# giuspugl/COSMOMAP2

Hardware: NVIDIA B200
Metric: tod_samples_per_s_per_pcg_iter (higher is better)
Workload: dtype f64

## Files before the change

### cosmomap2_b200/_cabi.py

```python
import ctypes
import os

_HERE = os.path.dirname(os.path.abspath(__file__))
LIB_PATH = os.environ.get("CM2_LIB") or os.path.join(_HERE, "csrc", "libcosmomap2_b200.so")

_vp = ctypes.c_void_p
_i64 = ctypes.c_int64
_int = ctypes.c_int
_f64 = ctypes.c_double

SIGNATURES = {
    "cm2_version": (_int, []),
    "cm2_last_error": (ctypes.c_char_p, []),
    "cm2_device_info": (_int, [ctypes.POINTER(_int), ctypes.POINTER(_i64), ctypes.POINTER(_int)]),
    "cm2_launch_count": (_i64, []),
    "cm2_pointing_apply": (_int, [_vp, _vp, _vp, _i64, _int, _vp, _vp, _vp]),
    "cm2_pointing_apply_t": (_int, [_vp, _vp, _vp, _i64, _int, _vp, _vp, _i64, _vp]),
    "cm2_pointing_apply_t_sorted": (_int, [_vp, _vp, _vp, _vp, _int, _vp, _vp, _i64, _vp]),
    "cm2_hits_i64": (_int, [_vp, _i64, _i64, _vp, _vp]),
    "cm2_angles": (_int, [_vp, _i64, _vp, _vp, _vp]),
    "cm2_pix_narrow": (_int, [_vp, _i64, _vp, _vp]),
    "cm2_pix_widen": (_int, [_vp, _i64, _vp, _vp]),
    "cm2_weights_moments": (_int, [_vp, _vp, _vp, _vp, _vp, _i64, _i64, _vp, _i64, _int, _vp, _i64, _vp]),
    "cm2_weights_moments_sorted": (_int, [_vp, _vp, _vp, _vp, _vp, _vp, _i64, _i64, _vp, _int, _vp, _i64, _vp]),
    "cm2_weights_mask": (_int, [_vp, _i64, _int, _f64, _vp, _vp]),
    "cm2_scan_scratch_bytes": (_i64, [_i64]),
    "cm2_weights_old2new": (_int, [_vp, _i64, _vp, _vp, _vp, _vp]),
    "cm2_compact_rows_f64": (_int, [_vp, _vp, _i64, _int, _vp, _vp]),
    "cm2_compact_rows_i64": (_int, [_vp, _vp, _i64, _int, _vp, _vp]),
    "cm2_relabel": (_int, [_vp, _i64, _vp, _vp]),
    "cm2_bd_build": (_int, [_vp, _i64, _int, _vp, _vp]),
    "cm2_bd_apply": (_int, [_vp, _i64, _int, _vp, _vp, _vp]),
    "cm2_bdfwd_apply": (_int, [_vp, _i64, _int, _vp, _vp, _vp]),
    "cm2_noise_white_apply": (_int, [_vp, _i64, _i64, _vp, _vp, _vp, _i64, _vp]),
    "cm2_toeplitz_scratch_bytes": (_i64, [_i64]),
    "cm2_noise_toeplitz_apply": (_int, [_vp, _int, _i64, _i64, _vp, _vp, _vp, _i64, _vp, _vp]),
    "cm2_toeplitz_fft_points": (_int, []),
    "cm2_toeplitz_fft_scratch_bytes": (_i64, [_i64]),
    "cm2_noise_toeplitz_fft_apply": (_int, [_vp, _int, _i64, _i64, _vp, _vp, _vp, _i64, _vp, _int, _int, _vp]),
    "cm2_filter_offset_apply": (_int, [_vp, _vp, _vp, _i64, _vp, _vp, _i64, _vp]),
    "cm2_amatvec_white": (_int, [_vp, _vp, _vp, _i64, _int, _vp, _i64, _i64, _vp, _vp, _vp, _i64, _i64, _vp]),
    "cm2_amatvec_white_set_stage": (_int, [_int]),
    "cm2_amatvec_filter": (_int, [_vp, _vp, _vp, _i64, _int, _vp, _vp, _i64, _vp, _vp, _i64, _vp]),
    "cm2_filter_runs_mark": (_int, [_vp, _vp, _vp, _i64, _i64, _vp, _vp, _vp]),
    "cm2_filter_runs_fill": (_int, [_vp, _vp, _vp, _int, _vp, _vp, _i64, _vp, _vp, _vp, _vp, _vp, _vp]),
    "cm2_filter_seg_mean": (_int, [_vp, _vp, _vp, _vp, _i64, _int, _vp, _vp, _vp]),
    "cm2_amatvec_filter_mu": (_int, [_vp, _vp, _vp, _i64, _int, _vp, _vp, _vp, _vp, _vp, _i64, _vp, _vp, _i64, _i64, _vp]),
    "cm2_filter_poly_gram": (_int, [_vp, _vp, _vp, _i64, _int, _vp, _vp, _vp]),
    "cm2_filter_poly_runs_fill": (_int, [_vp, _vp, _vp, _int, _vp, _vp, _i64, _int, _vp, _vp, _vp, _vp, _vp, _vp]),
    "cm2_filter_poly_seg_coef": (_int, [_vp, _vp, _vp, _vp, _i64, _int, _int, _vp, _vp, _vp, _vp]),
    "cm2_amatvec_filter_poly_mu": (_int, [_vp, _vp, _vp, _i64, _int, _vp, _vp, _vp, _vp, _vp, _i64, _int, _vp, _vp,
                                          _i64, _int, _i64, _vp]),
    "cm2_pointing_filter_mu": (_int, [_vp, _vp, _vp, _i64, _int, _vp, _vp, _vp, _vp, _vp, _i64, _vp, _vp, _vp]),
    "cm2_amatvec_toeplitz_max_band": (_int, []),
    "cm2_amatvec_toeplitz": (_int, [_vp, _vp, _vp, _i64, _int, _vp, _int, _i64, _i64, _vp, _vp, _vp, _i64, _vp]),
    "cm2_filter_poly_max_order": (_int, []),
    "cm2_filter_poly_set_tma": (_int, [_int]),
    "cm2_filter_poly_apply": (_int, [_vp, _vp, _vp, _i64, _i64, _int, _int, _vp, _vp, _i64, _vp]),
    "cm2_amatvec_filter_poly_max_order": (_int, []),
    "cm2_amatvec_filter_poly": (_int, [_vp, _vp, _vp, _i64, _int, _vp, _vp, _i64, _i64, _int, _vp, _vp, _i64, _vp]),
    "cm2_ground_filter_apply": (_int, [_vp, _i64, _i64, _vp, _vp, _vp, _vp, _vp]),
    "cm2_ground_filter_sub": (_int, [_vp, _i64, _i64, _vp, _vp, _vp, _vp, _vp]),
    "cm2_reorganize_map": (_int, [_vp, _vp, _i64, _int, _i64, _vp, _vp]),
    "cm2_defl_work_doubles": (_i64, [_int]),
    "cm2_defl_zt_apply": (_int, [_vp, _i64, _int, _i64, _vp, _int, _i64, _vp, _vp, _vp]),
    "cm2_defl_z_apply": (_int, [_vp, _i64, _int, _i64, _vp, _f64, _f64, _vp, _vp, _vp]),
    "cm2_coarse_apply": (_int, [_vp, _int, _vp, _vp, _vp]),
    "cm2_m2_apply": (_int, [_vp, _vp, _i64, _int, _i64, _vp, _vp, _i64, _int, _vp, _vp, _vp, _vp]),
    "cm2_m2_banded_apply": (_int, [_vp, _vp, _int, _vp, _vp, _i64, _int, _vp, _vp, _vp, _vp]),
    "cm2_dense_gram_work_doubles": (_i64, []),
    "cm2_dense_gram": (_int, [_vp, _i64, _int, _vp, _i64, _int, _i64, _vp, _i64, _vp, _vp]),
    "cm2_dense_combine": (_int, [_vp, _i64, _i64, _int, _vp, _i64, _int, _vp, _i64, _vp]),
    "cm2_dot": (_int, [_vp, _vp, _i64, _vp, _vp]),
    "cm2_axpby": (_int, [_f64, _vp, _f64, _vp, _i64, _vp]),
    "cm2_pcg_reset": (_int, [_vp, _i64, _vp, _f64, _vp]),
    "cm2_pcg_update_p": (_int, [_vp, _vp, _vp, _i64, _vp, _vp]),
    "cm2_pcg_update_xr": (_int, [_vp, _vp, _vp, _vp, _i64, _vp, _vp]),
    "cm2_pcg_bd_reset": (_int, [_vp, _i64, _int, _vp, _vp, _vp, _f64, _f64, _vp, _vp, _vp, _vp]),
    "cm2_pcg_bd_iter": (_int, [_vp, _i64, _int, _vp, _vp, _vp, _vp, _vp, _vp, _vp]),
    "cm2_pcg_bd_update_p": (_int, [_vp, _vp, _i64, _vp, _vp]),
    "cm2_pcg_bd_update": (_int, [_vp, _i64, _int, _vp, _vp, _vp, _vp, _vp, _vp, _vp]),
    "cm2_allreduce_p2p_signal_bytes": (_i64, []),
    "cm2_allreduce_p2p": (_int, [_vp, _vp, _vp, _int, _int, _i64, ctypes.c_uint32, _vp]),
    "cm2_enable_peer_access": (_int, [_int]),
    "cm2_allreduce_p2p_set_timeout": (_f64, [_f64]),
    "cm2_pcg_bd_iter_refuse": (_int, [_int]),
    "cm2_pcg_bd_iter_max_npix": (_i64, [_int]),
    "cm2_pcg_bd_tail_strided": (_int, [_int]),
    "cm2_pcg_sharded_signal_bytes": (_i64, []),
    "cm2_pcg_sharded_work_doubles": (_i64, []),
    "cm2_pcg_bd_sharded": (_int, [_int, _int, _int, _int, _int, _vp, _vp, _vp, _vp, _vp, _vp, _vp, _vp, _vp, _vp, _vp,
                                  _vp, ctypes.c_uint32, _f64, _f64, _f64, _vp]),
}

# ... 46 lines not shown
```

### cosmomap2_b200/csrc/tod_pass.cu

```cuda
#include <cstdint>
#include <type_traits>

#include "cm2_common.cuh"

namespace cm2 {

constexpr int K = 8;
constexpr int TILE = 32 * K;
constexpr int BLOCK = 256;
constexpr unsigned FULL = 0xffffffffu;

struct BlockW {
    const double *w;
    int64_t nblocks;
    int64_t blocksize;
    const int64_t *start;
    uint64_t magic;
};

static BlockW make_blockw(const double *w, int64_t nblocks, int64_t blocksize, const int64_t *start) {
    BlockW bw{w, nblocks, blocksize, start, 0};
    if (start == nullptr && blocksize > 1) bw.magic = ~(uint64_t)0 / (uint64_t)blocksize + 1;
    return bw;
}
// ... 41 lines not shown
    __device__ __forceinline__ int64_t tile(int64_t v) const {
        if (S == 1) return v;
        const unsigned q = (unsigned)v / S, r = (unsigned)v - q * S;
        return (int64_t)r * T + q;
    }
    __device__ __forceinline__ int64_t next(int64_t v, int64_t step, int64_t ntiles, int64_t &t) const {
        const int64_t nv = count();
        for (; v < nv; v += step) {
            t = tile(v);
            if (t < ntiles) return v;
        }
        t = -1;
        return v;
    }
};

static TileOrder make_order(int64_t nt, int64_t nstreams) {
    const int64_t ntiles = (nt + TILE - 1) / TILE;
    TileOrder o{1u, (unsigned)ntiles};
    if (nstreams > 1 && nstreams <= 65536 && ntiles >= 4 * nstreams && ntiles < ((int64_t)1 << 31)) {
        o.S = (unsigned)nstreams;
        o.T = (unsigned)((ntiles + nstreams - 1) / nstreams);
    }
    return o;
}

enum Cache { STREAM, KEEP };

template <Cache CP = STREAM>
__device__ __forceinline__ void load_pix(const int32_t *__restrict__ pix, int64_t t0, int64_t nt, int (&p)[K]) {
    if (t0 + K <= nt) {
        I8 v = CP == KEEP ? ld_keep_i8(pix + t0) : ld_stream_i8(pix + t0);
#pragma unroll
        for (int j = 0; j < K; ++j) p[j] = v.v[j];
    } else {
#pragma unroll
        for (int j = 0; j < K; ++j) p[j] = (t0 + j < nt) ? (CP == KEEP ? pix[t0 + j] : ld_stream_i1(pix + t0 + j)) : -1;
    }
}

template <Cache CP = STREAM>
__device__ __forceinline__ void load_f64(const double *__restrict__ a, int64_t t0, int64_t nt, double (&c)[K]) {
    if (t0 + K <= nt) {
        D4 v0 = CP == KEEP ? ld_keep_d4(a + t0) : ld_stream_d4(a + t0);
        D4 v1 = CP == KEEP ? ld_keep_d4(a + t0 + 4) : ld_stream_d4(a + t0 + 4);
#pragma unroll
        for (int j = 0; j < 4; ++j) { c[j] = v0.v[j]; c[4 + j] = v1.v[j]; }
    } else {
#pragma unroll
        for (int j = 0; j < K; ++j) c[j] = (t0 + j < nt) ? (CP == KEEP ? a[t0 + j] : ld_stream_d1(a + t0 + j)) : 0.0;
    }
}

template <int POL, Cache CP = STREAM>
__device__ __forceinline__ void load_tod(const int32_t *__restrict__ pix, const double *__restrict__ cs,
                                         const double *__restrict__ sn, int64_t t0, int64_t nt, int (&p)[K],
                                         double (&c)[K], double (&s)[K]) {
    load_pix<CP>(pix, t0, nt, p);
    if (POL > 1) { load_f64<CP>(cs, t0, nt, c); load_f64<CP>(sn, t0, nt, s); }
}

template <int POL>
__device__ __forceinline__ void gather_x(const double *__restrict__ x, const int (&p)[K], double (&xv)[K][POL]) {
#pragma unroll
    for (int j = 0; j < K; ++j) {
        const bool nw = (j == 0) || (p[j] != p[j - 1]);
#pragma unroll
        for (int k = 0; k < POL; ++k) xv[j][k] = 0.0;
        if (nw && p[j] >= 0) {
            const double *xp = x + (int64_t)POL * p[j];
#pragma unroll
            for (int k = 0; k < POL; ++k) xv[j][k] = __ldg(xp + k);
        }
    }
#pragma unroll
    for (int j = 1; j < K; ++j) {
        if (p[j] == p[j - 1]) {
#pragma unroll
            for (int k = 0; k < POL; ++k) xv[j][k] = xv[j - 1][k];
        }
    }
}

template <int POL>
__device__ __forceinline__ double project(const double (&xv)[POL], double c, double s) {
    if constexpr (POL == 1) return xv[0];
    else if constexpr (POL == 2) return fma(xv[1], s, xv[0] * c);
    else return fma(xv[2], s, fma(xv[1], c, xv[0]));
}

template <int POL>
__device__ __forceinline__ double project(const double (&xv)[K][POL], const double (&c)[K], const double (&s)[K], int j) {
    return project<POL>(xv[j], POL > 1 ? c[j] : 0.0, POL > 1 ? s[j] : 0.0);
}

template <int POL>
__device__ __forceinline__ auto pt_contrib(const double (&v)[K], const double (&c)[K], const double (&s)[K]) {
    return [&v, &c, &s](int j, double (&o)[POL]) {
        if constexpr (POL == 1) { o[0] = v[j]; }
        else if constexpr (POL == 2) { o[0] = v[j] * c[j]; o[1] = v[j] * s[j]; }
        else { o[0] = v[j]; o[1] = v[j] * c[j]; o[2] = v[j] * s[j]; }
    };
}

template <int NV, int STRIDE>
__device__ __forceinline__ void emit(double *__restrict__ y, int pix, const double (&v)[NV]) {
    if (pix >= 0) {
        double *dst = y + (int64_t)STRIDE * pix;
#pragma unroll
        for (int k = 0; k < NV; ++k) atomicAdd(dst + k, v[k]);
    }
}
// ... 87 lines not shown
__device__ __forceinline__ void run_scatter(double *__restrict__ y, const int (&p)[K], F contrib) {
    RunState<NV> rs;
    run_compress<NV, STRIDE>(y, p, contrib, rs);
    run_merge<NV, STRIDE>(y, rs);
}

template <int POL>
__global__ void __launch_bounds__(BLOCK) k_pointing_apply(const int32_t *__restrict__ pix, const double *__restrict__ cs,
                                                          const double *__restrict__ sn, int64_t nt,
                                                          const double *__restrict__ x, double *__restrict__ d) {
    const int lane = threadIdx.x & 31;
    const int64_t nwarps = (int64_t)gridDim.x * (BLOCK / 32);
    const int64_t ntiles = (nt + TILE - 1) / TILE;
    for (int64_t tile = (int64_t)blockIdx.x * (BLOCK / 32) + (threadIdx.x >> 5); tile < ntiles; tile += nwarps) {
        const int64_t t0 = tile * TILE + (int64_t)lane * K;
        if (t0 >= nt) continue;
        int p[K];
        double c[K], s[K], xv[K][POL], out[K];
        load_tod<POL>(pix, cs, sn, t0, nt, p, c, s);
        gather_x<POL>(x, p, xv);
#pragma unroll
        for (int j = 0; j < K; ++j) out[j] = p[j] >= 0 ? project<POL>(xv, c, s, j) : 0.0;
        if (t0 + K <= nt) {
            D4 a, b;
#pragma unroll
            for (int j = 0; j < 4; ++j) { a.v[j] = out[j]; b.v[j] = out[4 + j]; }
            st_stream_d4(d + t0, a);
            st_stream_d4(d + t0 + 4, b);
        } else {
#pragma unroll
            for (int j = 0; j < K; ++j) if (t0 + j < nt) d[t0 + j] = out[j];
        }
    }
}

template <int POL>
__global__ void __launch_bounds__(BLOCK) k_pointing_apply_t(const int32_t *__restrict__ pix, const double *__restrict__ cs,
                                                            const double *__restrict__ sn, int64_t nt,
                                                            const double *__restrict__ d, double *__restrict__ y) {
    const int lane = threadIdx.x & 31;
    const int64_t nwarps = (int64_t)gridDim.x * (BLOCK / 32);
    const int64_t ntiles = (nt + TILE - 1) / TILE;
    for (int64_t tile = (int64_t)blockIdx.x * (BLOCK / 32) + (threadIdx.x >> 5); tile < ntiles; tile += nwarps) {
        const int64_t t0 = tile * TILE + (int64_t)lane * K;
        int p[K];
        double c[K], s[K], v[K];
        load_pix(pix, t0, nt, p);
        load_f64(d, t0, nt, v);
        if (POL > 1) { load_f64(cs, t0, nt, c); load_f64(sn, t0, nt, s); }
        run_scatter<POL, POL>(y, p, pt_contrib<POL>(v, c, s));
    }
}

template <int POL, bool ILV, bool WS = false>
__global__ void __launch_bounds__(BLOCK) k_amatvec_white(const int32_t *__restrict__ pix, const double *__restrict__ cs,
                                                         const double *__restrict__ sn, int64_t nt, BlockW bw, TileOrder ord,
                                                         const double *__restrict__ x, double *__restrict__ y) {
    const int lane = threadIdx.x & 31;
    const int64_t nwarps = (int64_t)gridDim.x * (BLOCK / 32);
    const int64_t ntiles = (nt + TILE - 1) / TILE;
    RunState<POL> rs = RunState<POL>::empty();
    const int64_t nv = ILV ? ord.count() : ntiles;
    for (int64_t vt = (int64_t)blockIdx.x * (BLOCK / 32) + (threadIdx.x >> 5); vt < nv; vt += nwarps) {
        int64_t tile = vt;
        if constexpr (ILV) {
            tile = ord.tile(vt);
            if (tile >= ntiles) continue;
        }
        const int64_t t0 = tile * TILE + (int64_t)lane * K;
        int p[K];
        double c[K], s[K];
        load_tod<POL>(pix, cs, sn, t0, nt, p, c, s);
        run_merge<POL, POL>(y, rs);
        double w[K], xv[K][POL], v[K];
        if constexpr (WS) load_f64(bw.w, t0, nt, w);
        gather_x<POL>(x, p, xv);
        if constexpr (!WS) chunk_weights(bw, t0 < nt ? t0 : nt - 1, nt, w);
#pragma unroll
        for (int j = 0; j < K; ++j) v[j] = w[j] * project<POL>(xv, c, s, j);
        run_compress<POL, POL>(y, p, pt_contrib<POL>(v, c, s), rs);
    }
    run_merge<POL, POL>(y, rs);
}

template <int POL>
__device__ __forceinline__ void stage_flush(double *__restrict__ sm, double *__restrict__ y, int64_t base, int len) {
    const int lane = threadIdx.x & 31;
    __syncwarp();
    for (int i = lane; i < len; i += 32) {
        const double v = sm[i];
        if (v != 0.0) {
            sm[i] = 0.0;
            atomicAdd(y + base + i, v);
        }
    }
    __syncwarp();
}

template <int POL>
__global__ void __launch_bounds__(BLOCK) k_amatvec_white_staged(const int32_t *__restrict__ pix, const double *__restrict__ cs,
                                                                const double *__restrict__ sn, int64_t nt, BlockW bw, TileOrder ord,
                                                                const double *__restrict__ x, double *__restrict__ y, int wpix) {
    extern __shared__ double stage_sm[];
    const int lane = threadIdx.x & 31;
    double *sm = stage_sm + (size_t)(threadIdx.x >> 5) * POL * wpix;
    for (int i = lane; i < POL * wpix; i += 32) sm[i] = 0.0;
    __syncwarp();
    const int64_t nwarps = (int64_t)gridDim.x * (BLOCK / 32);
    const int64_t ntiles = (nt + TILE - 1) / TILE;
    const int64_t nv = ord.count();
    int64_t base_prev = 0;
    int len_prev = 0;
    for (int64_t vt = (int64_t)blockIdx.x * (BLOCK / 32) + (threadIdx.x >> 5); vt < nv; vt += nwarps) {
        const int64_t tile = ord.tile(vt);
        if (tile >= ntiles) continue;
        const int64_t t0 = tile * TILE + (int64_t)lane * K;
        int p[K];
        double c[K], s[K];
        load_tod<POL>(pix, cs, sn, t0, nt, p, c, s);
        if (len_prev) stage_flush<POL>(sm, y, base_prev, len_prev);
        len_prev = 0;
        double w[K], xv[K][POL], v[K];
        gather_x<POL>(x, p, xv);
        chunk_weights(bw, t0 < nt ? t0 : nt - 1, nt, w);
#pragma unroll
        for (int j = 0; j < K; ++j) v[j] = w[j] * project<POL>(xv, c, s, j);
        int lo = INT32_MAX, hi = INT32_MIN;
#pragma unroll
        for (int j = 0; j < K; ++j) {
            if (p[j] >= 0) { lo = min(lo, p[j]); hi = max(hi, p[j]); }
        }
        lo = __reduce_min_sync(FULL, lo);
        hi = __reduce_max_sync(FULL, hi);
        if (hi < lo) continue;
        auto contrib = pt_contrib<POL>(v, c, s);
// ... 719 lines not shown
}

static int check_tod(const void *pix, const void *c, const void *s, int64_t nt, int pol) {
    if (nt < 0) return set_error(CM2_ERR_ARG, "nt < 0");
    if (pol < 1 || pol > 3) return set_error(CM2_ERR_ARG, "No valid polarization key set! pol=%d (1=I, 2=QU, 3=IQU)", pol);
    if (nt > 0 && pix == nullptr) return set_error(CM2_ERR_ARG, "pix is NULL");
    if (pol > 1 && nt > 0 && (c == nullptr || s == nullptr)) return set_error(CM2_ERR_ARG, "cos/sin required for pol>1");
    if (!aligned(pix, 32) || !aligned(c, 32) || !aligned(s, 32))
        return set_error(CM2_ERR_ARG, "TOD arrays must be 32-byte aligned");
    return CM2_OK;
}

}

using namespace cm2;

extern "C" int cm2_pointing_apply(const int32_t *pix, const double *c, const double *s, int64_t nt, int pol,
                                  const double *x, double *d, cm2_stream_t stream) {
    int rc = check_tod(pix, c, s, nt, pol);
    if (rc) return rc;
    CM2_REQUIRE(aligned(d, 32), "d must be 32-byte aligned");
    if (nt == 0) return CM2_OK;
    cudaStream_t st = as_stream(stream);
    return with_pol(pol, [&](auto P) { return launch_tod(k_pointing_apply<P>, tod_blocks(nt), 0, st, pix, c, s, nt, x, d); });
}

extern "C" int cm2_pointing_apply_t(const int32_t *pix, const double *c, const double *s, int64_t nt, int pol,
                                    const double *d, double *y, int64_t npix, cm2_stream_t stream) {
    int rc = check_tod(pix, c, s, nt, pol);
    if (rc) return rc;
    CM2_REQUIRE(aligned(d, 32), "d must be 32-byte aligned");
    CM2_REQUIRE(npix >= 0, "npix < 0");
    cudaStream_t st = as_stream(stream);
    CM2_CUDA(zero_fill(y, npix, pol, st));
    if (nt == 0 || npix == 0) return CM2_OK;
    return with_pol(pol, [&](auto P) { return launch_tod(k_pointing_apply_t<P>, tod_blocks(nt), 0, st, pix, c, s, nt, d, y); });
}

static int check_blocks(const double *wblk, int64_t nblocks, int64_t blocksize, const int64_t *blk_start) {
    if (wblk == nullptr) return CM2_OK;
    if (nblocks <= 0) return set_error(CM2_ERR_ARG, "nblocks must be > 0 when weights are given");
    if (blk_start == nullptr && blocksize <= 0) return set_error(CM2_ERR_ARG, "blocksize must be > 0");
    return CM2_OK;
}

static int g_white_stage_wpix = 0;

extern "C" int cm2_amatvec_white_set_stage(int wpix) {
    CM2_REQUIRE(wpix >= 0 && wpix <= 1024, "stage window must be 0..1024 pixels");
    g_white_stage_wpix = wpix;
    return CM2_OK;
}

extern "C" int cm2_amatvec_white(const int32_t *pix, const double *c, const double *s, int64_t nt, int pol,
                                 const double *wblk, int64_t nblocks, int64_t blocksize, const int64_t *blk_start,
                                 const double *x, double *y, int64_t npix, int64_t nstreams, cm2_stream_t stream) {
    int rc = check_tod(pix, c, s, nt, pol);
    if (rc) return rc;
    rc = check_blocks(wblk, nblocks, blocksize, blk_start);
    if (rc) return rc;
    CM2_REQUIRE(npix >= 0, "npix < 0");
    cudaStream_t st = as_stream(stream);
    CM2_CUDA(zero_fill(y, npix, pol, st));
    if (nt == 0 || npix == 0) return CM2_OK;
    const BlockW bw = make_blockw(wblk, nblocks, blocksize, blk_start);
    const TileOrder ord = make_order(nt, nstreams);
    if (g_white_stage_wpix > 0) {
        const int wpix = g_white_stage_wpix;
        const size_t smem = sizeof(double) * (size_t)(BLOCK / 32) * pol * wpix;
        return with_pol(pol, [&](auto P) {
            return launch_tod(k_amatvec_white_staged<P>, tod_blocks(nt), smem, st, pix, c, s, nt, bw, ord, x, y, wpix);
        });
    }
    if (wblk != nullptr && blk_start == nullptr && blocksize == 1) {
        CM2_REQUIRE(nblocks >= nt && aligned(wblk, 32), "per-sample weights: nt values, 32-byte aligned");
        return with_pol(pol, [&](auto P) {
            return launch_tod(k_amatvec_white<P, false, true>, tod_blocks(nt), 0, st, pix, c, s, nt, bw, ord, x, y);
        });
    }
    return with_pol(pol, [&](auto P) {
        return launch_tod(ord.S > 1 ? k_amatvec_white<P, true> : k_amatvec_white<P, false>, tod_blocks(nt), 0, st,
                          pix, c, s, nt, bw, ord, x, y);
    });
}

template <int POL, int NLAG>
static int launch_amatvec_toeplitz(const int32_t *pix, const double *c, const double *s, int64_t nt, const ToepW &tw,
                                   const double *x, double *y, cudaStream_t st) {
    constexpr int VAL = TILE - 2 * ((NLAG + K - 1) / K) * K;
    return launch_tod(k_amatvec_toeplitz<POL, NLAG>, tod_blocks(nt, VAL), 0, st, pix, c, s, nt, tw, x, y);
}

template <int POL>
static int dispatch_amatvec_toeplitz(const int32_t *pix, const double *c, const double *s, int64_t nt, const ToepW &tw,
                                     const double *x, double *y, cudaStream_t st) {
    const int nlag = tw.nband - 1;
    if (nlag <= 2) return launch_amatvec_toeplitz<POL, 2>(pix, c, s, nt, tw, x, y, st);
    if (nlag <= 4) return launch_amatvec_toeplitz<POL, 4>(pix, c, s, nt, tw, x, y, st);
    return launch_amatvec_toeplitz<POL, 8>(pix, c, s, nt, tw, x, y, st);
}

extern "C" int cm2_amatvec_toeplitz_max_band(void) { return 9; }

extern "C" int cm2_amatvec_toeplitz(const int32_t *pix, const double *c, const double *s, int64_t nt, int pol,
                                    const double *band, int nband, int64_t nblocks, int64_t blocksize,
                                    const int64_t *blk_start, const double *x, double *y, int64_t npix,
                                    cm2_stream_t stream) {
    int rc = check_tod(pix, c, s, nt, pol);
    if (rc) return rc;
    CM2_REQUIRE(band != nullptr && nband >= 1, "band required");
    rc = check_blocks(band, nblocks, blocksize, blk_start);
    if (rc) return rc;
    if (nband > cm2_amatvec_toeplitz_max_band())
        return set_error(CM2_ERR_UNSUPPORTED, "fused Toeplitz A-matvec: nband=%d, bands of up to %d coefficients are supported",
                         nband, cm2_amatvec_toeplitz_max_band());
    CM2_REQUIRE(npix >= 0, "npix < 0");
    cudaStream_t st = as_stream(stream);
    CM2_CUDA(zero_fill(y, npix, pol, st));
    if (nt == 0 || npix == 0) return CM2_OK;
    const ToepW tw{band, nband, make_blockw(nullptr, nblocks, blocksize, blk_start)};
    return with_pol(pol, [&](auto P) { return dispatch_amatvec_toeplitz<P>(pix, c, s, nt, tw, x, y, st); });
}

extern "C" int cm2_weights_moments(const int32_t *pix, const double *c, const double *s, const double *w,
                                   const double *wblk, int64_t nblocks, int64_t blocksize, const int64_t *blk_start,
                                   int64_t nt, int pol, double *mom, int64_t npix, cm2_stream_t stream) {
    int rc = check_tod(pix, c, s, nt, pol);
    if (rc) return rc;
    rc = check_blocks(wblk, nblocks, blocksize, blk_start);
    if (rc) return rc;
    CM2_REQUIRE(aligned(w, 32), "w must be 32-byte aligned");
    CM2_REQUIRE(npix >= 0, "npix < 0");
    cudaStream_t st = as_stream(stream);
    CM2_CUDA(zero_fill(mom, npix, 6, st));
    if (nt == 0 || npix == 0) return CM2_OK;
    const BlockW bw = make_blockw(wblk, nblocks, blocksize, blk_start);
// ... 117 lines not shown
```

### cosmomap2_b200/linearoperators.py

```python
import numpy as np
import torch
from scipy.linalg import eigh, lu_factor, lu_solve

from . import _device as dv
from . import linop as lp
from .process_ces import BlockWeights, ProcessTimeSamples


def _stream():
    return dv.stream()


class SparseLO(lp.LinearOperator):

    def __init__(self, n, m, pix_samples, pol=1, angle_processed=None):
        dv.require_cuda()
        self.ncols = int(n)
        self.nrows = int(m)
        self.pol = pol
        self.pairs = pix_samples
        if pol not in (1, 2, 3):
            raise RuntimeError("No valid polarization key set!\t=>\tpol=%d \n \
                                    Possible values are pol=%d(I),%d(QU), %d(IQU)." % (pol, 1, 2, 3))
        if len(pix_samples) != self.nrows:
# ... 428 lines not shown
                self.nseg, self._max_seg_len, self.poly_order, int(self._sorted), dv.ptr(d), dv.ptr(out),
                d.numel(), _stream())
        return out

    def mult(self, d):
        if FILTER_STAGED:
            return self._staged(d)
        out = torch.empty_like(d)
        dv.call("cm2_filter_offset_apply", dv.ptr(self._pix_dev), dv.ptr(self._seg_start), dv.ptr(self._seg_end),
                self.nseg, dv.ptr(d), dv.ptr(out), d.numel(), _stream())
        return out

    def polyfilter(self, d):
        return self._staged(d)

    polyfilter_multithreads = polyfilter

    def compute_legendres(self):
        from .utilities import get_legendre_polynomials
        sizes = []
        for array in self.subscans:
            for i in array:
                if int(i) not in sizes:
                    sizes.append(int(i))
        self._legendres = {size: get_legendre_polynomials(self.poly_order, size) for size in sizes}

    @property
    def legendres(self):
        if self._legendres is None:
            self.compute_legendres()
        return self._legendres


TOD_INTERLEAVE_MIN_MAP_BYTES = 100e6


def _tod_streams(P, samples_per_timeline):
    ns = int(samples_per_timeline or 0)
    if ns <= 0 or 2 * 8 * P.pol * P.ncols < TOD_INTERLEAVE_MIN_MAP_BYTES:
        return 1
    k = P.nrows // ns
    return int(k) if k > 1 and k * ns == P.nrows else 1


def _filter_timeline(F):
    ns = np.atleast_1d(np.asarray(F.nsamples)).astype(np.int64)
    return int(ns[0]) if ns.size and np.all(ns == ns[0]) else 0


WHITE_STAGE_RUN_RANGE = (3.0, 6.0)
WHITE_STAGE_MIN_CONTIGUITY = 0.9
WHITE_STAGE_WINDOW = 288
WHITE_SORT_BELOW_RUN = 3.0


class _FusedWhiteA(lp.LinearOperator):

    def __init__(self, P, N):
        self.P, self.N = P, N
        n = P.pol * P.ncols
        bs = N._blk.blocksize if N is not None else 0
        self._streams = _tod_streams(P, bs)
        self._mode = None
        self._sorted = None
        super(_FusedWhiteA, self).__init__(n, n, matvec=self._run, symmetric=True, device=True)

    def _choose(self):
        run, contig = self.P.run_statistics()
        if run < WHITE_SORT_BELOW_RUN and self.P.nrows > 0:
            self._mode = "sorted"
            self._build_sorted()
        elif WHITE_STAGE_RUN_RANGE[0] <= run < WHITE_STAGE_RUN_RANGE[1] and contig >= WHITE_STAGE_MIN_CONTIGUITY:
            self._mode = "staged"
        else:
            self._mode = "registers"

    def _build_sorted(self):
        P, N = self.P, self.N
        order = torch.sort(P._pix_dev, stable=True).indices
        nflag = int((P._pix_dev < 0).sum().item())
        order = order[nflag:]
        nts = int(order.numel())
        pad = (-nts) % 8
        pix = torch.full((nts + pad,), -1, dtype=torch.int32, device=order.device)
        pix[:nts] = P._pix_dev[order]
        cs = sn = None
        if P.pol > 1:
            cs, sn = dv.zeros_f64(nts + pad), dv.zeros_f64(nts + pad)
            cs[:nts] = P._cos_dev[order]
            sn[:nts] = P._sin_dev[order]
        w = None
        if N is not None:
            starts = dv.to_dev(N._blk.starts, torch.int64)
            blk = torch.bucketize(order, starts[1:], right=True)
            w = dv.zeros_f64(nts + pad)
            w[:nts] = N.weights_dev()[blk]
        self._sorted = (pix, cs, sn, w, nts + pad)

    def _run(self, x):
        P = self.P
        if self._mode is None:
            self._choose()
        y = dv.out_f64(P.ncols * P.pol)
        if self._mode == "sorted":
            pix, cs, sn, w, nts = self._sorted
            dv.call("cm2_amatvec_white", dv.ptr(pix), dv.ptr(cs), dv.ptr(sn), nts, P.pol,
                    dv.ptr(w) if w is not None else None, nts if w is not None else 0, 1, None, dv.ptr(x), dv.ptr(y),
                    P.ncols, 1, _stream())
            return y
        if self.N is None:
            w, nb, bs, startp = None, 0, 0, None
        else:
            w = dv.ptr(self.N.weights_dev())
            nb, bs, startp = self.N._blk.args()
        if self._mode == "staged":
            dv.call("cm2_amatvec_white_set_stage", WHITE_STAGE_WINDOW)
        try:
            dv.call("cm2_amatvec_white", dv.ptr(P._pix_dev), dv.ptr(P._cos_dev), dv.ptr(P._sin_dev), P.nrows, P.pol,
                    w, nb, bs, startp, dv.ptr(x), dv.ptr(y), P.ncols, self._streams, _stream())
        finally:
            if self._mode == "staged":
                dv.call("cm2_amatvec_white_set_stage", 0)
        return y


FILTER_RUN_TABLE = True


def _tile_tables(seg_start, seg_end, nseg, nt):
    dev = seg_start.device
    ntiles = (nt + 255) // 256
    tile_t0 = torch.arange(ntiles, dtype=torch.int64, device=dev) * 256
    tile_seg = torch.searchsorted(seg_end, tile_t0, right=True)
    kk = torch.clamp(tile_seg, max=nseg - 1)
    a, b = seg_start[kk], seg_end[kk]
    t1 = torch.clamp(tile_t0 + 256, max=nt)
    inside = (tile_seg < nseg) & (a <= tile_t0) & (t1 <= b)
    outside = (tile_seg >= nseg) | (a >= t1)
    tile_flag = torch.full((ntiles,), 2, dtype=torch.uint8, device=dev)
    tile_flag[inside] = 1
    tile_flag[outside] = 0
    return tile_seg.to(torch.int32), tile_flag


def _build_filter_runs(P, F):
    nt, st = P.nrows, _stream()
    dev = P._pix_dev.device
    ss, se = F._seg_start_host, F._seg_end_host
    if F.nseg == 0 or np.any(ss[1:] < se[:-1]):
        return False
    flags = torch.empty(max(nt, 1), dtype=torch.int32, device=dev)
    pixm = torch.empty(max(nt, 1), dtype=torch.int32, device=dev)
    dv.call("cm2_filter_runs_mark", dv.ptr(P._pix_dev), dv.ptr(F._seg_start), dv.ptr(F._seg_end), F.nseg, nt,
            dv.ptr(flags), dv.ptr(pixm), st)
    runidx = torch.empty(max(nt, 1), dtype=torch.int32, device=dev)
    count = torch.zeros(1, dtype=torch.int64, device=dev)
    scratch = torch.empty(int(dv.call("cm2_scan_scratch_bytes", nt)) // 8 + 1, dtype=torch.int64, device=dev)
    dv.call("cm2_weights_old2new", dv.ptr(flags), nt, dv.ptr(runidx), dv.ptr(count), dv.ptr(scratch), st)
    nruns = int(count.item())
    del flags, scratch
    if nruns == 0 or 2 * nruns > nt:
        return False
    run_pix = torch.empty(nruns, dtype=torch.int32, device=dev)
    run_mom = torch.empty(3 * nruns, dtype=torch.float64, device=dev)
    seg_first = torch.empty(max(F.nseg, 1), dtype=torch.int64, device=dev)
    seg_nruns = torch.empty(max(F.nseg, 1), dtype=torch.int32, device=dev)
    dv.call("cm2_filter_runs_fill", dv.ptr(pixm), dv.ptr(P._cos_dev), dv.ptr(P._sin_dev), P.pol,
            dv.ptr(F._seg_start), dv.ptr(F._seg_end), F.nseg, dv.ptr(runidx), dv.ptr(run_pix), dv.ptr(run_mom),
            dv.ptr(seg_first), dv.ptr(seg_nruns), st)
    del pixm, runidx
    tile_seg, tile_flag = _tile_tables(F._seg_start, F._seg_end, F.nseg, nt)
    mu = torch.empty(max(F.nseg, 1), dtype=torch.float64, device=dev)
# ... 541 lines not shown
```

### cosmomap2_b200/workloads.py

```python
import time

import numpy as np
import torch
import torch.distributed as dist


def _world():
    if dist.is_available() and dist.is_initialized():
        return dist.get_world_size(), dist.get_rank()
    return 1, 0


def _max_over_ranks(v):
    t = torch.tensor([float(v)], dtype=torch.float64, device="cuda")
    if _world()[0] > 1:
        dist.all_reduce(t, op=dist.ReduceOp.MAX)
    return float(t.item())


def _barrier():
    torch.cuda.synchronize()
    if _world()[0] > 1:
        dist.barrier()
        torch.cuda.synchronize()
# ... 295 lines not shown
    x_m2, _res, out["M_2lvl"] = _solve(cm, A, b, M2, rtol, maxiter)
    out["iteration_ratio"] = out["M_2lvl"]["iterations"] / max(out["M_BD"]["iterations"], 1)
    out["build_plus_solve_vs_M_BD_solve"] = (out["deflation"]["build_seconds"] + out["M_2lvl"]["seconds"]) / out["M_BD"]["seconds"]
    ax1, ax2 = A._apply(x_bd), A._apply(x_m2)
    out["Ax_agreement"] = float(torch.linalg.norm(ax1 - ax2) / torch.linalg.norm(ax1))
    for k in ("M_BD", "M_2lvl"):
        out[k]["samples_per_s_per_pcg_iter"] = nt * world / (out[k]["ms_per_iteration"] * 1e-3)
    al_ms = time_device(lambda: A_local._apply(x_bd), time_iters)
    m2_ms = time_device(lambda: M2._apply(x_bd), time_iters)
    out["A_local_apply_ms"] = al_ms
    out["M_2lvl_apply_ms"] = m2_ms
    out["roofline"] = _roofline("k_seg_mean + k_amatvec_filter_mu (P^T F P, cm2_amatvec_filter_mu)" if poly_order == 0
                                else "P^T F_K P (Legendre order %d)" % poly_order, 20.0 * nt + 48.0 * npix, al_ms,
                                note=("DRAM traffic of the pair measured by ncu at 1e8 samples, 8 samples per pixel crossing "
                                      "(profiles/r02_filter_mu_ncu.txt): 2.41 GB against 2.024 GB algorithmic -- k_amatvec_filter_mu "
                                      "reads 1.00x its 20 B/sample, the rest is the run table of k_seg_mean (28 B per run); "
                                      "not measured at this size, hence traffic = null") if poly_order == 0 else None)
    out["hbm_GB"] = torch.cuda.max_memory_allocated() / 1e9
    _close(A)
    return out


def white(nt=1e9, nside=2048, nx=3200, ny=1600, ndet=64, steps=30):
    import cosmomap2_b200 as cm
    from cosmomap2_b200 import distributed
    from cosmomap2_b200.pcg import make_solver
    world, rank = _world()
    pol = 3
    nt, ns, pix, phi, _sl, _ss, g = make_scan(int(nt), nside, nx, ny, ndet, 8.0, seed=rank, turnaround=0.0)
    npix_full = 12 * nside ** 2
    w = 0.5 + torch.rand(ndet, generator=g, device="cuda", dtype=torch.float64).cpu().numpy()
    N = cm.BlockLO(ns, w)
    pts = cm.ProcessTimeSamples(pix, npix_full, obspix=np.arange(npix_full), pol=pol, phi=phi, w=N.diag,
                                comm=(True if world > 1 else None))
    del phi
    npix = pts.get_new_pixel[0]
    n = pol * npix
    P = cm.SparseLO(npix, nt, pts._pix_dev, pol=pol, angle_processed=pts)
    Mbd = cm.BlockDiagonalPreconditionerLO(pts, npix, pol=pol)
    A_local = P.T * N * P
    A = distributed.AllReduceLO(A_local) if world > 1 else A_local
    b = torch.randn(n, dtype=torch.float64, device="cuda", generator=torch.Generator(device="cuda").manual_seed(5))
    b = A._apply(b)
    x, info = cm.cg(A, b, M=Mbd, rtol=1e-10, maxiter=20)
    relres = float(torch.linalg.norm(b - A._apply(x)) / torch.linalg.norm(b))
    solver = make_solver(A, Mbd, n)

    def one_step():
        solver.start(b)
        solver.step_async()
        solver.tick()
    it_ms = time_device(one_step, steps)
    al_ms = time_device(lambda: A_local._apply(x), steps)
    out = {"config": "configs[4]: white noise, IQU nside=%d, M_BD PCG" % nside, "world": world, "nt_total": nt * world,
           "nt_per_gpu": nt, "npix": int(npix), "nside": nside, "cg_info": int(info), "relres": relres,
           "ms_per_pcg_iteration": it_ms, "samples_per_s_per_pcg_iter": nt * world / (it_ms * 1e-3),
           "A_local_apply_ms": al_ms,
           "roofline": _roofline("k_amatvec_white<3> (cm2_amatvec_white)", 20.0 * nt + 48.0 * npix, al_ms),
           "solver": type(solver).__name__, "hbm_GB": torch.cuda.max_memory_allocated() / 1e9}
    _close(A)
    return out
```

### include/cosmomap2_b200.h

```cpp
#ifndef COSMOMAP2_B200_H
#define COSMOMAP2_B200_H

#include <stdint.h>

#ifdef __cplusplus
extern "C" {
#endif

#define CM2_OK 0
#define CM2_ERR_ARG (-1)
#define CM2_ERR_CUDA (-2)
#define CM2_ERR_UNSUPPORTED (-3)

typedef void *cm2_stream_t;

int cm2_version(void);
const char *cm2_last_error(void);
int cm2_device_info(int *sm_count, int64_t *l2_bytes, int *cc);
int64_t cm2_launch_count(void);

int cm2_pointing_apply(const int32_t *pix, const double *cos2phi, const double *sin2phi,
                       int64_t nt, int pol, const double *x, double *d, cm2_stream_t stream);
int cm2_pointing_apply_t(const int32_t *pix, const double *cos2phi, const double *sin2phi,
                         int64_t nt, int pol, const double *d, double *y, int64_t npix,
                         cm2_stream_t stream);
int cm2_pointing_apply_t_sorted(const int64_t *rowptr, const int32_t *perm,
                                const double *cos2phi, const double *sin2phi, int pol,
                                const double *d, double *y, int64_t npix, cm2_stream_t stream);
int cm2_hits_i64(const int32_t *pix, int64_t nt, int64_t npix, int64_t *hits,
                 cm2_stream_t stream);

int cm2_angles(const double *phi, int64_t nt, double *cos2phi, double *sin2phi,
               cm2_stream_t stream);
int cm2_pix_narrow(const int64_t *pix64, int64_t nt, int32_t *pix32, cm2_stream_t stream);
int cm2_pix_widen(const int32_t *pix32, int64_t nt, int64_t *pix64, cm2_stream_t stream);
int cm2_weights_moments(const int32_t *pix, const double *cos2phi, const double *sin2phi,
                        const double *w, const double *wblk, int64_t nblocks, int64_t blocksize,
                        const int64_t *blk_start, int64_t nt, int pol, double *mom, int64_t npix,
                        cm2_stream_t stream);
int cm2_weights_moments_sorted(const int64_t *rowptr, const int32_t *perm, const double *cos2phi,
                               const double *sin2phi, const double *w, const double *wblk,
                               int64_t nblocks, int64_t blocksize, const int64_t *blk_start,
                               int pol, double *mom, int64_t npix, cm2_stream_t stream);
int cm2_weights_mask(const double *mom, int64_t npix, int pol, double threshold_cond,
                     int32_t *good, cm2_stream_t stream);
int64_t cm2_scan_scratch_bytes(int64_t n);
int cm2_weights_old2new(const int32_t *good, int64_t npix, int32_t *old2new,
                        int64_t *npix_new_dev, void *scratch, cm2_stream_t stream);
int cm2_compact_rows_f64(const double *src, const int32_t *old2new, int64_t npix, int width,
                         double *dst, cm2_stream_t stream);
int cm2_compact_rows_i64(const int64_t *src, const int32_t *old2new, int64_t npix, int width,
                         int64_t *dst, cm2_stream_t stream);
int cm2_relabel(int32_t *pix, int64_t nt, const int32_t *old2new, cm2_stream_t stream);

int cm2_bd_build(const double *mom, int64_t npix, int pol, double *inv, cm2_stream_t stream);
int cm2_bd_apply(const double *inv, int64_t npix, int pol, const double *x, double *y,
                 cm2_stream_t stream);
int cm2_bdfwd_apply(const double *mom, int64_t npix, int pol, const double *x, double *y,
                    cm2_stream_t stream);

int cm2_noise_white_apply(const double *wblk, int64_t nblocks, int64_t blocksize,
                          const int64_t *blk_start, const double *d, double *out, int64_t nt,
                          cm2_stream_t stream);
int64_t cm2_toeplitz_scratch_bytes(int64_t nblocks);
int cm2_noise_toeplitz_apply(const double *band, int nband, int64_t nblocks, int64_t blocksize,
                             const int64_t *blk_start, const double *d, double *out, int64_t nt,
                             void *scratch, cm2_stream_t stream);
int cm2_toeplitz_fft_points(void);
int64_t cm2_toeplitz_fft_scratch_bytes(int64_t nblocks);
int cm2_noise_toeplitz_fft_apply(const double *coef, int nband, int64_t nblocks, int64_t blocksize,
                                 const int64_t *blk_start, const double *d, double *out,
                                 int64_t nt, void *scratch, int init, int pair, cm2_stream_t stream);
int cm2_filter_offset_apply(const int32_t *pix, const int64_t *seg_start, const int64_t *seg_end,
                            int64_t nseg, const double *d, double *out, int64_t nt,
                            cm2_stream_t stream);

int cm2_amatvec_white(const int32_t *pix, const double *cos2phi, const double *sin2phi,
                      int64_t nt, int pol, const double *wblk, int64_t nblocks,
                      int64_t blocksize, const int64_t *blk_start, const double *x, double *y,
                      int64_t npix, int64_t nstreams, cm2_stream_t stream);
int cm2_amatvec_white_set_stage(int wpix);
int cm2_amatvec_filter(const int32_t *pix, const double *cos2phi, const double *sin2phi,
                       int64_t nt, int pol, const int64_t *seg_start, const int64_t *seg_end,
                       int64_t nseg, const double *x, double *y, int64_t npix,
                       cm2_stream_t stream);

int cm2_filter_runs_mark(const int32_t *pix, const int64_t *seg_start, const int64_t *seg_end,
                         int64_t nseg, int64_t nt, int32_t *flags, int32_t *pix_masked,
                         cm2_stream_t stream);
int cm2_filter_runs_fill(const int32_t *pix_masked, const double *cos2phi, const double *sin2phi,
                         int pol, const int64_t *seg_start, const int64_t *seg_end, int64_t nseg,
                         const int32_t *runidx, int32_t *run_pix, double *run_mom,
                         int64_t *seg_first, int32_t *seg_nruns, cm2_stream_t stream);
int cm2_filter_seg_mean(const int32_t *run_pix, const double *run_mom, const int64_t *seg_first,
                        const int32_t *seg_nruns, int64_t nseg, int pol, const double *x,
                        double *mu, cm2_stream_t stream);
int cm2_amatvec_filter_mu(const int32_t *pix, const double *cos2phi, const double *sin2phi,
                          int64_t nt, int pol, const int64_t *seg_start, const int64_t *seg_end,
                          const double *seg_mu, const int32_t *tile_seg, const uint8_t *tile_flag,
                          int64_t nseg, const double *x, double *y, int64_t npix, int64_t nstreams,
                          cm2_stream_t stream);

int cm2_filter_poly_gram(const int32_t *pix, const int64_t *seg_start, const int64_t *seg_end,
                         int64_t nseg, int poly_order, double *W, double *info, cm2_stream_t stream);
int cm2_filter_poly_runs_fill(const int32_t *pix_masked, const double *cos2phi, const double *sin2phi,
                              int pol, const int64_t *seg_start, const int64_t *seg_end, int64_t nseg,
                              int poly_order, const int32_t *runidx, int32_t *run_pix, double *run_mom,
                              int64_t *seg_first, int32_t *seg_nruns, cm2_stream_t stream);
int cm2_filter_poly_seg_coef(const int32_t *run_pix, const double *run_mom, const int64_t *seg_first,
                             const int32_t *seg_nruns, int64_t nseg, int pol, int poly_order,
                             const double *W, const double *x, double *coef, cm2_stream_t stream);
int cm2_amatvec_filter_poly_mu(const int32_t *pix, const double *cos2phi, const double *sin2phi,
                               int64_t nt, int pol, const int64_t *seg_start, const int64_t *seg_end,
                               const double *seg_coef, const int32_t *tile_seg, const uint8_t *tile_flag,
                               int64_t nseg, int poly_order, const double *x, double *y, int64_t npix,
                               int accumulate, int64_t nstreams, cm2_stream_t stream);

int cm2_pointing_filter_mu(const int32_t *pix, const double *cos2phi, const double *sin2phi,
                           int64_t nt, int pol, const int64_t *seg_start, const int64_t *seg_end,
                           const double *seg_mu, const int32_t *tile_seg, const uint8_t *tile_flag,
                           int64_t nseg, const double *x, double *d, cm2_stream_t stream);

int cm2_amatvec_toeplitz_max_band(void);
int cm2_amatvec_toeplitz(const int32_t *pix, const double *cos2phi, const double *sin2phi,
                         int64_t nt, int pol, const double *band, int nband, int64_t nblocks,
                         int64_t blocksize, const int64_t *blk_start, const double *x, double *y,
                         int64_t npix, cm2_stream_t stream);

int64_t cm2_defl_work_doubles(int r);
int cm2_defl_zt_apply(const double *Z, int64_t n, int r, int64_t ldz, const double *X,
                      int ncols_x, int64_t ldx, double *out, double *work, cm2_stream_t stream);
int cm2_defl_z_apply(const double *Z, int64_t n, int r, int64_t ldz, const double *c,
                     double alpha, double beta, const double *y0, double *y,
// ... 76 lines not shown
```

Baseline: 243.1 billion.

## Pack pointing pixel indices into 8-byte words per lane for white matvec

Adds a one-time packing kernel that encodes each lane's K=8 pixel indices as a base, a 16-bit delta and 2-bit codes in one 64-bit word. Lanes that don't fit this encoding are marked as escapes and fall back to reading int32 pixels. The white-noise A matvec reads these packed words with an evict-first, L1 no-allocate streaming load and prefetches the next tile's word one iteration ahead. This cuts pixel-index HBM traffic from 4 to about 1 byte per sample, at the cost of decode ALU work and escape fallback reads. The packed path is only chosen for single-stream layouts with short runs and high contiguity.

```diff
diff --git a/cosmomap2_b200/_cabi.py b/cosmomap2_b200/_cabi.py
--- a/cosmomap2_b200/_cabi.py
+++ b/cosmomap2_b200/_cabi.py
@@ -39,7 +39,8 @@
     "cm2_toeplitz_fft_scratch_bytes": (_i64, [_i64]),
     "cm2_noise_toeplitz_fft_apply": (_int, [_vp, _int, _i64, _i64, _vp, _vp, _vp, _i64, _vp, _int, _int, _vp]),
     "cm2_filter_offset_apply": (_int, [_vp, _vp, _vp, _i64, _vp, _vp, _i64, _vp]),
-    "cm2_amatvec_white": (_int, [_vp, _vp, _vp, _i64, _int, _vp, _i64, _i64, _vp, _vp, _vp, _i64, _i64, _vp]),
+    "cm2_amatvec_white": (_int, [_vp, _vp, _vp, _vp, _i64, _int, _vp, _i64, _i64, _vp, _vp, _vp, _i64, _i64, _vp]),
+    "cm2_pack_pointing": (_int, [_vp, _i64, _vp, _vp, _vp]),
     "cm2_amatvec_white_set_stage": (_int, [_int]),
     "cm2_amatvec_filter": (_int, [_vp, _vp, _vp, _i64, _int, _vp, _vp, _i64, _vp, _vp, _i64, _vp]),
     "cm2_filter_runs_mark": (_int, [_vp, _vp, _vp, _i64, _i64, _vp, _vp, _vp]),
diff --git a/cosmomap2_b200/csrc/tod_pass.cu b/cosmomap2_b200/csrc/tod_pass.cu
--- a/cosmomap2_b200/csrc/tod_pass.cu
+++ b/cosmomap2_b200/csrc/tod_pass.cu
@@ -117,12 +117,71 @@
     }
 }
 
+constexpr int PK_FLAGGED = -1, PK_ESCAPE = -2;
+
+__device__ __forceinline__ uint64_t ld_stream_u64(const uint64_t *p) {
+    uint64_t pol, r;
+    asm("createpolicy.fractional.L2::evict_first.b64 %0, 1.0;" : "=l"(pol));
+    asm volatile("ld.global.L1::no_allocate.L2::cache_hint.b64 %0, [%1], %2;" : "=l"(r) : "l"(p), "l"(pol));
+    return r;
+}
+
+__device__ __forceinline__ uint64_t load_packed(const uint64_t *__restrict__ pk, int64_t t0, int64_t nt) {
+    return t0 + K <= nt ? ld_stream_u64(pk + t0 / K) : (uint64_t)(uint32_t)PK_ESCAPE;
+}
+
+__device__ __forceinline__ void unpack_pix(uint64_t wd, const int32_t *__restrict__ pix, int64_t t0, int64_t nt,
+                                           int (&p)[K]) {
+    const int b0 = (int)(uint32_t)wd;
+    if (b0 == PK_ESCAPE) {
+        load_pix(pix, t0, nt, p);
+        return;
+    }
+    const int b1 = b0 + (int)(int16_t)(uint16_t)(wd >> 32);
+    const unsigned codes = (unsigned)(wd >> 48);
+#pragma unroll
+    for (int j = 0; j < K; ++j) {
+        const unsigned code = (codes >> (2 * j)) & 3u;
+        p[j] = ((code & 2u) ? b1 : b0) + (int)(code & 1u);
+    }
+}
+
 template <int POL, Cache CP = STREAM>
 __device__ __forceinline__ void load_tod(const int32_t *__restrict__ pix, const double *__restrict__ cs,
                                          const double *__restrict__ sn, int64_t t0, int64_t nt, int (&p)[K],
                                          double (&c)[K], double (&s)[K]) {
     load_pix<CP>(pix, t0, nt, p);
     if (POL > 1) { load_f64<CP>(cs, t0, nt, c); load_f64<CP>(sn, t0, nt, s); }
+}
+
+__device__ __forceinline__ uint64_t pack_lane(const int (&q)[K]) {
+    bool all_flagged = true, any_flagged = false;
+    int b0 = q[0];
+#pragma unroll
+    for (int j = 0; j < K; ++j) {
+        all_flagged &= q[j] == -1;
+        any_flagged |= q[j] < 0;
+        b0 = min(b0, q[j]);
+    }
+    if (all_flagged) return (uint32_t)PK_FLAGGED;
+    if (any_flagged) return (uint32_t)PK_ESCAPE;
+    int b1 = b0;
+#pragma unroll
+    for (int j = 0; j < K; ++j) {
+        if (q[j] - b0 > 1 && (b1 == b0 || q[j] < b1)) b1 = q[j];
+    }
+    if (b1 - b0 > INT16_MAX) return (uint32_t)PK_ESCAPE;
+    uint64_t codes = 0;
+#pragma unroll
+    for (int j = 0; j < K; ++j) {
+        const int d0 = q[j] - b0, d1 = q[j] - b1;
+        unsigned code;
+        if (d0 <= 1) code = (unsigned)d0;
+        else if (d1 <= 1) code = 2u + (unsigned)d1;
+        else return (uint32_t)PK_ESCAPE;
+        codes |= (uint64_t)code << (2 * j);
+    }
+    return (uint64_t)(uint32_t)b0 | ((uint64_t)(uint16_t)(b1 - b0) << 32) | (codes << 48);
 }
 
 template <int POL>
@@ -316,16 +375,26 @@
     }
 }
 
-template <int POL, bool ILV, bool WS = false>
+template <int POL, bool ILV, bool WS = false, bool PK = false>
 __global__ void __launch_bounds__(BLOCK) k_amatvec_white(const int32_t *__restrict__ pix, const double *__restrict__ cs,
                                                          const double *__restrict__ sn, int64_t nt, BlockW bw, TileOrder ord,
-                                                         const double *__restrict__ x, double *__restrict__ y) {
+                                                         const double *__restrict__ x, double *__restrict__ y,
+                                                         const uint64_t *__restrict__ pk) {
     const int lane = threadIdx.x & 31;
     const int64_t nwarps = (int64_t)gridDim.x * (BLOCK / 32);
     const int64_t ntiles = (nt + TILE - 1) / TILE;
     RunState<POL> rs = RunState<POL>::empty();
     const int64_t nv = ILV ? ord.count() : ntiles;
-    for (int64_t vt = (int64_t)blockIdx.x * (BLOCK / 32) + (threadIdx.x >> 5); vt < nv; vt += nwarps) {
+    const int64_t vt0 = (int64_t)blockIdx.x * (BLOCK / 32) + (threadIdx.x >> 5);
+    uint64_t wd_next = 0;
+    if constexpr (PK) wd_next = load_packed(pk, (ILV ? ord.tile(vt0) : vt0) * TILE + (int64_t)lane * K, nt);
+    for (int64_t vt = vt0; vt < nv; vt += nwarps) {
+        uint64_t wd = 0;
+        if constexpr (PK) {
+            wd = wd_next;
+            const int64_t vn = vt + nwarps;
+            wd_next = load_packed(pk, vn < nv ? (ILV ? ord.tile(vn) : vn) * TILE + (int64_t)lane * K : nt, nt);
+        }
         int64_t tile = vt;
         if constexpr (ILV) {
             tile = ord.tile(vt);
@@ -334,8 +403,13 @@
         const int64_t t0 = tile * TILE + (int64_t)lane * K;
         int p[K];
         double c[K], s[K];
-        load_tod<POL>(pix, cs, sn, t0, nt, p, c, s);
+        if constexpr (PK) {
+            if (POL > 1) { load_f64(cs, t0, nt, c); load_f64(sn, t0, nt, s); }
+        } else {
+            load_tod<POL>(pix, cs, sn, t0, nt, p, c, s);
+        }
         run_merge<POL, POL>(y, rs);
+        if constexpr (PK) unpack_pix(wd, pix, t0, nt, p);
         double w[K], xv[K][POL], v[K];
         if constexpr (WS) load_f64(bw.w, t0, nt, w);
         gather_x<POL>(x, p, xv);
@@ -345,6 +419,23 @@
         run_compress<POL, POL>(y, p, pt_contrib<POL>(v, c, s), rs);
     }
     run_merge<POL, POL>(y, rs);
+}
+
+__global__ void __launch_bounds__(BLOCK) k_pack_pointing(const int32_t *__restrict__ pix, int64_t nt,
+                                                         uint64_t *__restrict__ packed, unsigned long long *__restrict__ nescape) {
+    const int64_t nlanes = (nt + K - 1) / K;
+    unsigned nesc = 0;
+    for (int64_t l = (int64_t)blockIdx.x * BLOCK + threadIdx.x; l < nlanes; l += (int64_t)gridDim.x * BLOCK) {
+        uint64_t wd = (uint32_t)PK_ESCAPE;
+        if (l * K + K <= nt) {
+            const I8 v = ld_stream_i8(pix + l * K);
+            wd = pack_lane(v.v);
+        }
+        nesc += (int)(uint32_t)wd == PK_ESCAPE;
+        packed[l] = wd;
+    }
+    nesc = __reduce_add_sync(FULL, nesc);
+    if ((threadIdx.x & 31) == 0 && nesc) atomicAdd(nescape, (unsigned long long)nesc);
 }
 
 template <int POL>
@@ -1170,20 +1261,23 @@
     return CM2_OK;
 }
 
-extern "C" int cm2_amatvec_white(const int32_t *pix, const double *c, const double *s, int64_t nt, int pol,
-                                 const double *wblk, int64_t nblocks, int64_t blocksize, const int64_t *blk_start,
-                                 const double *x, double *y, int64_t npix, int64_t nstreams, cm2_stream_t stream) {
+extern "C" int cm2_amatvec_white(const int32_t *pix, const uint64_t *pix_packed, const double *c, const double *s,
+                                 int64_t nt, int pol, const double *wblk, int64_t nblocks, int64_t blocksize,
+                                 const int64_t *blk_start, const double *x, double *y, int64_t npix, int64_t nstreams,
+                                 cm2_stream_t stream) {
     int rc = check_tod(pix, c, s, nt, pol);
     if (rc) return rc;
     rc = check_blocks(wblk, nblocks, blocksize, blk_start);
     if (rc) return rc;
     CM2_REQUIRE(npix >= 0, "npix < 0");
+    CM2_REQUIRE(aligned(pix_packed, 8), "pix_packed must be 8-byte aligned");
     cudaStream_t st = as_stream(stream);
     CM2_CUDA(zero_fill(y, npix, pol, st));
     if (nt == 0 || npix == 0) return CM2_OK;
     const BlockW bw = make_blockw(wblk, nblocks, blocksize, blk_start);
     const TileOrder ord = make_order(nt, nstreams);
     if (g_white_stage_wpix > 0) {
+        CM2_REQUIRE(pix_packed == nullptr, "the staged scatter reads int32 pixels only");
         const int wpix = g_white_stage_wpix;
         const size_t smem = sizeof(double) * (size_t)(BLOCK / 32) * pol * wpix;
         return with_pol(pol, [&](auto P) {
@@ -1192,14 +1286,27 @@
     }
     if (wblk != nullptr && blk_start == nullptr && blocksize == 1) {
         CM2_REQUIRE(nblocks >= nt && aligned(wblk, 32), "per-sample weights: nt values, 32-byte aligned");
+        CM2_REQUIRE(pix_packed == nullptr, "per-sample weights read int32 pixels only");
         return with_pol(pol, [&](auto P) {
-            return launch_tod(k_amatvec_white<P, false, true>, tod_blocks(nt), 0, st, pix, c, s, nt, bw, ord, x, y);
+            return launch_tod(k_amatvec_white<P, false, true>, tod_blocks(nt), 0, st, pix, c, s, nt, bw, ord, x, y,
+                              (const uint64_t *)nullptr);
         });
     }
     return with_pol(pol, [&](auto P) {
-        return launch_tod(ord.S > 1 ? k_amatvec_white<P, true> : k_amatvec_white<P, false>, tod_blocks(nt), 0, st,
-                          pix, c, s, nt, bw, ord, x, y);
+        auto kern = ord.S > 1 ? (pix_packed ? k_amatvec_white<P, true, false, true> : k_amatvec_white<P, true>)
+                              : (pix_packed ? k_amatvec_white<P, false, false, true> : k_amatvec_white<P, false>);
+        return launch_tod(kern, tod_blocks(nt), 0, st, pix, c, s, nt, bw, ord, x, y, pix_packed);
     });
+}
+
+extern "C" int cm2_pack_pointing(const int32_t *pix, int64_t nt, uint64_t *packed, int64_t *nescape, cm2_stream_t stream) {
+    CM2_REQUIRE(nt >= 0, "nt < 0");
+    CM2_REQUIRE(nescape != nullptr && (nt == 0 || (pix != nullptr && packed != nullptr)), "NULL argument");
+    CM2_REQUIRE(aligned(pix, 32) && aligned(packed, 8), "pix must be 32-byte and packed 8-byte aligned");
+    cudaStream_t st = as_stream(stream);
+    CM2_CUDA(zero_fill(nescape, 1, 1, st));
+    if (nt == 0) return CM2_OK;
+    return launch_tod(k_pack_pointing, tod_blocks(nt), 0, st, pix, nt, packed, reinterpret_cast<unsigned long long *>(nescape));
 }
 
 template <int POL, int NLAG>
diff --git a/cosmomap2_b200/linearoperators.py b/cosmomap2_b200/linearoperators.py
--- a/cosmomap2_b200/linearoperators.py
+++ b/cosmomap2_b200/linearoperators.py
@@ -504,6 +504,7 @@
 WHITE_STAGE_MIN_CONTIGUITY = 0.9
 WHITE_STAGE_WINDOW = 288
 WHITE_SORT_BELOW_RUN = 3.0
+WHITE_PACK_BELOW_RUN = 16.0
 
 
 class _FusedWhiteA(lp.LinearOperator):
@@ -515,6 +516,8 @@
         self._streams = _tod_streams(P, bs)
         self._mode = None
         self._sorted = None
+        self._packed = None
+        self.nescape = 0
         super(_FusedWhiteA, self).__init__(n, n, matvec=self._run, symmetric=True, device=True)
 
     def _choose(self):
@@ -526,6 +529,22 @@
             self._mode = "staged"
         else:
             self._mode = "registers"
+            if self._streams == 1 and run < WHITE_PACK_BELOW_RUN and contig >= WHITE_STAGE_MIN_CONTIGUITY:
+                self._build_packed()
+
+    def _build_packed(self):
+        P = self.P
+        self._packed = torch.empty(max((P.nrows + 7) // 8, 1), dtype=torch.int64, device=P._pix_dev.device)
+        nesc = torch.empty(1, dtype=torch.int64, device=P._pix_dev.device)
+        dv.call("cm2_pack_pointing", dv.ptr(P._pix_dev), P.nrows, dv.ptr(self._packed), dv.ptr(nesc), _stream())
+        self.nescape = int(nesc.item())
+
+    def tod_bytes(self):
+        if self._mode is None:
+            self._choose()
+        if self._packed is not None:
+            return 17 * self.P.nrows + 32 * self.nescape
+        return 20 * self.P.nrows
 
     def _build_sorted(self):
         P, N = self.P, self.N
@@ -556,7 +575,7 @@
         y = dv.out_f64(P.ncols * P.pol)
         if self._mode == "sorted":
             pix, cs, sn, w, nts = self._sorted
-            dv.call("cm2_amatvec_white", dv.ptr(pix), dv.ptr(cs), dv.ptr(sn), nts, P.pol,
+            dv.call("cm2_amatvec_white", dv.ptr(pix), None, dv.ptr(cs), dv.ptr(sn), nts, P.pol,
                     dv.ptr(w) if w is not None else None, nts if w is not None else 0, 1, None, dv.ptr(x), dv.ptr(y),
                     P.ncols, 1, _stream())
             return y
@@ -568,8 +587,9 @@
         if self._mode == "staged":
             dv.call("cm2_amatvec_white_set_stage", WHITE_STAGE_WINDOW)
         try:
-            dv.call("cm2_amatvec_white", dv.ptr(P._pix_dev), dv.ptr(P._cos_dev), dv.ptr(P._sin_dev), P.nrows, P.pol,
-                    w, nb, bs, startp, dv.ptr(x), dv.ptr(y), P.ncols, self._streams, _stream())
+            dv.call("cm2_amatvec_white", dv.ptr(P._pix_dev), dv.ptr(self._packed),
+                    dv.ptr(P._cos_dev), dv.ptr(P._sin_dev), P.nrows, P.pol, w, nb, bs, startp, dv.ptr(x), dv.ptr(y),
+                    P.ncols, self._streams, _stream())
         finally:
             if self._mode == "staged":
                 dv.call("cm2_amatvec_white_set_stage", 0)
diff --git a/cosmomap2_b200/workloads.py b/cosmomap2_b200/workloads.py
--- a/cosmomap2_b200/workloads.py
+++ b/cosmomap2_b200/workloads.py
@@ -371,11 +371,14 @@
         solver.tick()
     it_ms = time_device(one_step, steps)
     al_ms = time_device(lambda: A_local._apply(x), steps)
+    from cosmomap2_b200 import linearoperators as lo
+    fused = [f for f in A_local.planned() if isinstance(f, lo._FusedWhiteA)]
+    tod_bytes = fused[0].tod_bytes() if fused else 20.0 * nt
     out = {"config": "configs[4]: white noise, IQU nside=%d, M_BD PCG" % nside, "world": world, "nt_total": nt * world,
            "nt_per_gpu": nt, "npix": int(npix), "nside": nside, "cg_info": int(info), "relres": relres,
            "ms_per_pcg_iteration": it_ms, "samples_per_s_per_pcg_iter": nt * world / (it_ms * 1e-3),
            "A_local_apply_ms": al_ms,
-           "roofline": _roofline("k_amatvec_white<3> (cm2_amatvec_white)", 20.0 * nt + 48.0 * npix, al_ms),
+           "roofline": _roofline("k_amatvec_white<3> (cm2_amatvec_white)", tod_bytes + 48.0 * npix, al_ms),
            "solver": type(solver).__name__, "hbm_GB": torch.cuda.max_memory_allocated() / 1e9}
     _close(A)
     return out
diff --git a/include/cosmomap2_b200.h b/include/cosmomap2_b200.h
--- a/include/cosmomap2_b200.h
+++ b/include/cosmomap2_b200.h
@@ -75,10 +75,11 @@
                             int64_t nseg, const double *d, double *out, int64_t nt,
                             cm2_stream_t stream);
 
-int cm2_amatvec_white(const int32_t *pix, const double *cos2phi, const double *sin2phi,
-                      int64_t nt, int pol, const double *wblk, int64_t nblocks,
+int cm2_amatvec_white(const int32_t *pix, const uint64_t *pix_packed, const double *cos2phi,
+                      const double *sin2phi, int64_t nt, int pol, const double *wblk, int64_t nblocks,
                       int64_t blocksize, const int64_t *blk_start, const double *x, double *y,
                       int64_t npix, int64_t nstreams, cm2_stream_t stream);
+int cm2_pack_pointing(const int32_t *pix, int64_t nt, uint64_t *packed, int64_t *nescape, cm2_stream_t stream);
 int cm2_amatvec_white_set_stage(int wpix);
 int cm2_amatvec_filter(const int32_t *pix, const double *cos2phi, const double *sin2phi,
                        int64_t nt, int pol, const int64_t *seg_start, const int64_t *seg_end,
```

Measured after the change: 255.5 billion, median of 6. 5.1% higher.
